# tohinz/multiple-objects-gan

Measured on AMD Instinct MI355X. Metric: images/sec per G+D train step, 256x256 coco-attngan, higher is better.
Workload: dtype f32

## Files before the change

include/mogan_hip.h:

```cpp
#ifndef MOGAN_HIP_H
#define MOGAN_HIP_H

#include <stddef.h>
#include <stdint.h>

#ifdef __cplusplus
extern "C" {
#endif

typedef struct ihipStream_t* hipStream_t;

#define MOGAN_ERR_SHAPE (-1)
#define MOGAN_ERR_LAUNCH (-2)
#define MOGAN_ERR_WS (-3)

#define MOGAN_ACT_NONE 0
#define MOGAN_ACT_RELU 1
#define MOGAN_ACT_LRELU 2
#define MOGAN_ACT_GLU 3
#define MOGAN_ACT_TANH 4
#define MOGAN_ACT_SIGMOID 5

int mogan_abi_version(void);
int mogan_gemm_set_split_target(int blocks);
// ... 82 lines not shown

size_t mogan_pk_panel_bytes(int B, int C, int HW);
int mogan_deep_block_eligible(int B, int Cin, int Hs, int Ws, int Cout, int KH, int KW, int stride, int ph, int pw, int act,
                              int groups);
int mogan_deep_conv_bn_act_fwd(const float* x, const void* xpanel, const void* wpk, const float* gamma, const float* beta,
                               float* rmean, float* rvar, float* y, float* stats, float* z, void* zpanel, int B, int Cin, int Hs,
                               int Ws, int Cout, int KH, int KW, int stride, int ph, int pw, float eps, float momentum, int act,
                               float slope, int groups, void* ws, size_t ws_bytes, hipStream_t stream);
int mogan_deep_conv_bn_act_bwd(const float* dz, const float* y, const float* stats, const float* gamma, const float* beta,
                               const void* wpk_dgrad, float* dy, float* dgamma, float* dbeta, int accumulate, float* dx, int B,
                               int Cin, int Hs, int Ws, int Cout, int KH, int KW, int stride, int ph, int pw, int act, float slope,
                               int groups, void* ws, size_t ws_bytes, hipStream_t stream);

typedef struct MoganPkArgs {
    const void* wpk; const void* panel; float* raw;
    int B, M;
    int Cp, CGp, cg0;
    int PH, PW, outH, outW;
    int KH, KW, stride, ph, pw, dgrad;
    int nsplit;
} MoganPkArgs;
#define MOGAN_TAIL_MAXSRC 3
typedef struct MoganTailArgs {
    const float* src[MOGAN_TAIL_MAXSRC]; long long src_bs[MOGAN_TAIL_MAXSRC]; long long src_slab[MOGAN_TAIL_MAXSRC];
    int src_nsplit[MOGAN_TAIL_MAXSRC]; int nsrc;
    const float* add; long long add_bs;
    const float* mask; long long mask_bs;
    const float* scale; const float* shift;
    int relu, box;
    float* dst; long long dst_bs;
    void* panel; int CGp, cg0;
    int B, n, H, W;
} MoganTailArgs;
int mogan_pk_group(int n, MoganPkArgs* args, hipStream_t stream);
int mogan_panel_tail_group(int n, const MoganTailArgs* args, hipStream_t stream);

size_t mogan_upconv3x3_ws_bytes(int Cout, int Cin);
int mogan_upconv3x3_k4(const float* w, float* k4, int Cout, int Cin, hipStream_t stream);
int mogan_upconv3x3_k4_group(int n, const float* const* w, float* const* k4, const int* Cout, const int* Cin, hipStream_t stream);
int mogan_upconv3x3_fwd(const float* x, const float* w, float* y, int B, int Cin, int Hs, int Ws, int Cout, void* ws,
                        size_t ws_bytes, hipStream_t stream);
int mogan_upconv3x3_dgrad(const float* dy, const float* w, float* dx, int B, int Cin, int Hs, int Ws, int Cout, void* ws,
                          size_t ws_bytes, hipStream_t stream);
int mogan_upconv3x3_wgrad(const float* dy, const float* x, float* dw, int B, int Cin, int Hs, int Ws, int Cout,
                          int accumulate, void* ws, size_t ws_bytes, hipStream_t stream);
int mogan_down2_sum(const float* du, float* dx, int planes, int H, int W, hipStream_t stream);

int mogan_bmm(const float* a, const float* b, float* c, int batch, int M, int N, int K, long long sAb, long long sAm,
              long long sAk, long long sBb, long long sBk, long long sBn, long long sCb, long long sCm, long long sCn,
              int accumulate, void* ws, size_t ws_bytes, hipStream_t stream);

size_t mogan_bn_ws_bytes(int B, int C, int HW);
int mogan_bn_stats(const float* x, int B, int C, int HW, float eps, float momentum, float* mean, float* invstd,
                   float* running_mean, float* running_var, void* ws, size_t ws_bytes, hipStream_t stream);
int mogan_bn_act_fwd(const float* x, const float* mean, const float* invstd, const float* gamma, const float* beta,
                     const float* residual, float* y, int B, int C, int HW, int act, float slope, hipStream_t stream);
int mogan_bn_running_update(const float* mean, const float* invstd, float* running_mean, float* running_var, int C, long long n,
                            float eps, float momentum, hipStream_t stream);

int mogan_bn_act_fwd_fused(const float* x, const float* gamma, const float* beta, const float* residual, float* running_mean,
                           float* running_var, float* mean, float* invstd, float* y, int B, int C, int HW, int act, float slope,
                           float eps, float momentum, void* ws, size_t ws_bytes, hipStream_t stream);
int mogan_bn_act_grouped_eligible(int G, int B, int C, int HW);
int mogan_bn_act_grouped_fwd(const float* x, const float* gamma, const float* beta, float* running_mean, float* running_var, float* mean,
                             float* invstd, float* y, int G, int B, int C, int HW, int act, float slope, float eps, float momentum,
                             hipStream_t stream);
int mogan_bn_act_grouped_bwd(const float* x, const float* dy, const float* mean, const float* invstd, const float* gamma, const float* beta,
// ... 131 lines not shown
```

multiple-objects-gan_amd/csrc/mogan_pgemm.hip:

```cpp
#include <hip/hip_runtime.h>
#include <stdint.h>
#include <stdlib.h>
#include <algorithm>
#include "../../include/mogan_hip.h"
#include "mogan_internal.h"
#include "mogan_mma.h"
#include <type_traits>
#ifndef PK_NSET
#define PK_NSET 3
#endif
#define PK_TRIP (PK_NSET == 2 ? 2 : 6)

namespace {

typedef float f32x16 __attribute__((ext_vector_type(16)));

struct PkP {
    const unsigned char* A;
    const unsigned char* P;
    float* C; float* ws;
    int M, N, K;
    int Mt, KS;
    unsigned long long a_cls_stride;
    unsigned a_bytes, p_bytes;
    int ntile, kt_per, nsplit;
    long long slab;
    int accumulate;
    int dgrad, ncls;
    int Cc, CG;
    int CGp, cg0;
    int PH, PW;
    int RH, RW;
    int s, ph, pw, nkw;
    int outH, outW;
    int gx, gy;
};

__device__ __forceinline__ unsigned xcd_order(unsigned L, unsigned total) {
    const unsigned k = L & 7u, j = L >> 3, q = total >> 3, r = total & 7u;
    return k * q + (k < r ? k : r) + j;
}

__device__ __forceinline__ uint4 ldg16(__amdgpu_buffer_rsrc_t r, unsigned off, bool ok) {
    return __builtin_bit_cast(uint4, __builtin_amdgcn_raw_buffer_load_b128(r, ok ? off : 0xFFFFFFF0u, 0, 0));
}

template <int TM, int TN, int WM = 4>
__device__ __forceinline__ void pgemm_body(const PkP& p, unsigned V, const unsigned nblk) {
    constexpr int WN = 4 / WM;
    constexpr int BM = WM * TM * 32, BN = WN * TN * 32, RS = 208;
    constexpr int NCH = BN * 12 / 256;
    __shared__ __attribute__((aligned(16))) unsigned char Bs[2][BN * RS];

    const int tid = threadIdx.x, lane = tid & 63, wave = tid >> 6;
    const int wm = wave % WM, wn = wave / WM;
    V = xcd_order(V, nblk);
    const unsigned bx = V % p.gx; V /= p.gx;
    const unsigned cls = V % p.ncls; V /= p.ncls;
    const unsigned by = V % p.gy;
    const int sp = V / p.gy;
    const int n0 = bx * BN, m0 = by * BM;
    const int t_beg = sp * p.kt_per, t_end = min(p.ntile, t_beg + p.kt_per);

    const __amdgpu_buffer_rsrc_t rA = __builtin_amdgcn_make_buffer_rsrc((void*)(p.A + cls * p.a_cls_stride), (short)0,
                                                                         (int)p.a_bytes, 0x00020000);
    const __amdgpu_buffer_rsrc_t rP = __builtin_amdgcn_make_buffer_rsrc((void*)p.P, (short)0, (int)p.p_bytes, 0x00020000);

    int py = 0, px = 0, kh0 = 0, kw0 = 0;
    if (p.dgrad) { py = cls / p.s; px = cls % p.s; kh0 = (py + p.ph) % p.s; kw0 = (px + p.pw) % p.s; }
    const int RHW = p.RH * p.RW;
    int ry[NCH], rx[NCH]; unsigned pb[NCH]; unsigned ldso[NCH], cho[NCH]; bool rok[NCH];
#pragma unroll
    for (int i = 0; i < NCH; ++i) {
        const int c = tid + 256 * i, row = c / 12, ch = c - row * 12;
        const int n = n0 + row;
        rok[i] = n < p.N;
        const int nn = rok[i] ? n : 0;
        const int img = nn / RHW, rem = nn - img * RHW;
        const int r = rem / p.RW, cc = rem - r * p.RW;
        if (p.dgrad) { ry[i] = (r * p.s + py + p.ph - kh0) / p.s; rx[i] = (cc * p.s + px + p.pw - kw0) / p.s; }
        else { ry[i] = r * p.s - p.ph; rx[i] = cc * p.s - p.pw; }
        pb[i] = (unsigned)img * (unsigned)(p.PH * p.PW);
        ldso[i] = row * RS + ch * 16;
        cho[i] = ch * 16;
    }
// ... 116 lines not shown
        }
    }

    const bool split = p.nsplit > 1;
    float* __restrict__ slab = p.ws + (size_t)sp * p.slab;
    const bool addc = !split && p.accumulate;
    const size_t cms = (size_t)p.outH * p.outW;
#pragma unroll
    for (int tb = 0; tb < TN; ++tb) {
        const int n = n0 + (wn * TN + tb) * 32 + (lane & 31);
        const bool nok = n < p.N;
        const int nn = nok ? n : 0;
        const int img = nn / RHW, rem = nn - img * RHW;
        const int r = rem / p.RW, cc = rem - r * p.RW;
        const size_t pos = p.dgrad ? (size_t)(r * p.s + py) * p.outW + (cc * p.s + px) : (size_t)rem;
        const size_t cbase = (size_t)img * p.M * cms + pos;
#pragma unroll
        for (int ta = 0; ta < TM; ++ta) {
#pragma unroll
            for (int r16 = 0; r16 < 16; ++r16) {
                const int m = m0 + (wm * TM + ta) * 32 + (r16 & 3) + 8 * (r16 >> 2) + 4 * (lane >> 5);
                if (nok && m < p.M) {
                    float v = acc[ta][tb][r16];
                    float* dst = (split ? slab : p.C) + cbase + (size_t)m * cms;
                    if (addc) v += *dst;
                    *dst = v;
                }
            }
        }
    }
}

template <int TM, int TN, int OCC>
__global__ __launch_bounds__(256, OCC) void pgemm_kernel(const PkP p) { pgemm_body<TM, TN>(p, blockIdx.x, gridDim.x); }

constexpr int PK_MAXG = 8;
struct PkGroup { PkP p[PK_MAXG]; unsigned end[PK_MAXG]; int n; };

template <int TM, int TN, int OCC, int WM>
__global__ __launch_bounds__(256, OCC) void pgemm_group_kernel(const PkGroup g) {
    int pi = 0;
#pragma unroll
    for (int i = 0; i < PK_MAXG - 1; ++i) if (i + 1 < g.n && blockIdx.x >= g.end[i]) pi = i + 1;
    const unsigned start = pi ? g.end[pi - 1] : 0u;
    pgemm_body<TM, TN, WM>(g.p[pi], blockIdx.x - start, g.end[pi] - start);
}

__global__ __launch_bounds__(256) void apack_kernel(const float* __restrict__ x, unsigned char* __restrict__ P, int Bn, int C,
                                                    int HW) {
    __shared__ float L[32][65];
    const int tid = threadIdx.x;
    const long long Q = (long long)Bn * HW;
    const long long q0 = (long long)blockIdx.x * 64;
    const int c0 = blockIdx.y * 32;
#pragma unroll
    for (int j = 0; j < 8; ++j) {
        const int e = tid + 256 * j, cl = e >> 6, ql = e & 63;
        const long long q = q0 + ql;
        float v = 0.f;
        if (q < Q) {
            const long long img = q / HW, pix = q - img * HW;
            v = x[(img * C + c0 + cl) * HW + pix];
        }
        L[cl][ql] = v;
    }
    __syncthreads();
    const int ql = tid >> 2, g8 = tid & 3;
    const long long q = q0 + ql;
    if (q >= Q) return;
    uint32_t w[3][4];
#pragma unroll
    for (int j = 0; j < 4; ++j) x6_split2(L[g8 * 8 + 2 * j][ql], L[g8 * 8 + 2 * j + 1][ql], w[0][j], w[1][j], w[2][j]);
    unsigned char* d = P + ((size_t)q * (C >> 5) + blockIdx.y) * 192 + g8 * 16;
#pragma unroll
    for (int pl = 0; pl < 3; ++pl) *(uint4*)(d + pl * 64) = make_uint4(w[pl][0], w[pl][1], w[pl][2], w[pl][3]);
}

struct WpackP { const float* w; unsigned char* A; int Cout, Cin, KH, KW, s, ph, pw, dgrad, M, Cc, Mt, KS; unsigned long long cls_stride; };
// ... 377 lines not shown
           (act == MOGAN_ACT_NONE || act == MOGAN_ACT_RELU || act == MOGAN_ACT_LRELU);
}

static inline long long cdiv(long long a, long long b) { return (a + b - 1) / b; }
static inline size_t up256(size_t v) { return (v + 255) & ~(size_t)255; }

static int g_pk_force = 0;

struct PkGeom { int ncls, nkh, nkw, M, Cc, K, Mt, KS; unsigned long long cls_bytes; };

static bool pk_geom(int Cout, int Cin, int KH, int KW, int s, int dgrad, PkGeom& g) {
    if (Cout <= 0 || Cin <= 0 || KH <= 0 || KW <= 0 || s <= 0) return false;
    if (!dgrad) {
        if (Cin % 32) return false;
        g.ncls = 1; g.nkh = KH; g.nkw = KW; g.M = Cout; g.Cc = Cin;
    } else {
        if (Cout % 32 || KH % s || KW % s) return false;
        g.ncls = s * s; g.nkh = KH / s; g.nkw = KW / s; g.M = Cin; g.Cc = Cout;
    }
    if (KH * KW > 25) return false;
    g.K = g.nkh * g.nkw * g.Cc;
    g.Mt = (int)cdiv(g.M, 32); g.KS = g.K / 16;
    g.cls_bytes = (unsigned long long)g.Mt * g.KS * 3072ull;
    return g.cls_bytes < (1ull << 32);
}

struct PkCfg { int tm, tn; };
static const PkCfg kPk[] = {{1, 2}, {1, 4}, {2, 2}};
enum { NPK = 3 };
static int g_pk_cfg = -1, g_pk_split = 0;
#ifndef PK_OCC12
#define PK_OCC12 3
#endif
#ifndef PK_G64_OCC
#define PK_G64_OCC 2
#endif
static int g_pk_group_tile = -1;
static inline int a_prof_mode(int dgrad) { return dgrad ? 11 : 10; }

template <int TM, int TN, int OCC>
static void launch_pk(unsigned blocks, hipStream_t st, const PkP& p) {
    hipLaunchKernelGGL((pgemm_kernel<TM, TN, OCC>), dim3(blocks), dim3(256), 0, st, p);
}

static int run_pk(PkP& p, void* ws, size_t ws_bytes, int prof_mode, hipStream_t st, bool keep_slabs = false) {
    int best = 0; double bestw = 1e300;
    for (int c = 0; c < NPK; ++c) {
        const int bm = 128 * kPk[c].tm, bn = 32 * kPk[c].tn;
        double w = (double)cdiv(p.M, bm) * bm * (double)cdiv(p.N, bn) * bn;
        w *= c == 0 ? 1.0 : 1.15;
        if (w < bestw * 0.999) { bestw = w; best = c; }
    }
    if (g_pk_cfg >= 0) best = g_pk_cfg;
    const int bm = 128 * kPk[best].tm, bn = 32 * kPk[best].tn;
    p.gx = (int)cdiv(p.N, bn); p.gy = (int)cdiv(p.M, bm);
    const long long tiles = (long long)p.gx * p.gy * p.ncls;
    const long long c_numel = (long long)p.slab;
    int nsplit = 1;
    const int target = mogan_split_target(st);
    if (tiles < target && p.ntile >= 8) {
        nsplit = (int)cdiv(target, tiles);
        nsplit = std::min(nsplit, p.ntile / 4);
        if (nsplit < 1) nsplit = 1;
    }
    if (g_pk_split > 0) nsplit = std::min(g_pk_split, p.ntile);
    if (nsplit > 1) {
        const long long fit = ws ? (long long)(ws_bytes / (sizeof(float) * (size_t)c_numel)) : 0;
        if (fit < 2) nsplit = 1; else nsplit = (int)std::min<long long>(nsplit, fit);
    }
    p.kt_per = (int)cdiv(cdiv(p.ntile, nsplit), PK_TRIP) * PK_TRIP;
    p.nsplit = (int)cdiv(p.ntile, p.kt_per);
    p.ws = (float*)ws;
    const long long blocks = tiles * p.nsplit;
    if (blocks <= 0 || blocks > 0x7fffffff) return MOGAN_ERR_SHAPE;
    const double flops = 2.0 * (double)p.M * (double)p.N * p.ncls * (double)p.K;
    mogan_prof_begin(prof_mode, best, flops, p.M, p.N * p.ncls, p.K, st);
    switch (best) {
        case 1: launch_pk<1, 4, 2>((unsigned)blocks, st, p); break;
        case 2: launch_pk<2, 2, 2>((unsigned)blocks, st, p); break;
        default: launch_pk<1, 2, PK_OCC12>((unsigned)blocks, st, p); break;
    }
    mogan_prof_end(1, st);
    if (p.nsplit > 1 && !keep_slabs) mogan_splitk_reduce_dense((const float*)ws, p.C, c_numel, p.nsplit, p.accumulate, st);
    return hipGetLastError() == hipSuccess ? 0 : MOGAN_ERR_LAUNCH;
}

static int apack(const float* x, unsigned char* P, int B, int C, int HW, hipStream_t st) {
    const long long Q = (long long)B * HW;
    hipLaunchKernelGGL(apack_kernel, dim3((unsigned)cdiv(Q, 64), (unsigned)(C / 32)), dim3(256), 0, st, x, P, B, C, HW);
    return 0;
}

}

extern "C" {

int mogan_pk_debug_force(int take_all, int cfg, int split) {
    g_pk_force = take_all; g_pk_cfg = (cfg >= 0 && cfg < NPK) ? cfg : -1; g_pk_split = split > 0 ? split : 0;
    return 0;
}

int mogan_pk_conv_eligible(int B, int Cin, int Hs, int Ws, int Cout, int KH, int KW, int stride, int ph, int pw, int dgrad) {
    PkGeom g;
    if (B <= 0 || Hs <= 0 || Ws <= 0 || !pk_geom(Cout, Cin, KH, KW, stride, dgrad, g)) return 0;
    const int OH = (Hs + 2 * ph - KH) / stride + 1, OW = (Ws + 2 * pw - KW) / stride + 1;
    if (OH <= 0 || OW <= 0) return 0;
    if (dgrad && (Hs % stride || Ws % stride)) return 0;
    const long long pix = dgrad ? (long long)B * OH * OW : (long long)B * Hs * Ws;
    if (pix * g.Cc * 6 >= (1ll << 32)) return 0;
    if (g_pk_force) return 1;
    const int rows_hw = dgrad ? (Hs / stride) * (Ws / stride) : OH * OW;
    return rows_hw <= 64 && g.K >= 1024 && g.M >= 128;
}

size_t mogan_pk_weight_bytes(int Cout, int Cin, int KH, int KW, int stride, int dgrad) {
    PkGeom g;
    if (!pk_geom(Cout, Cin, KH, KW, stride, dgrad, g)) return 0;
    return (size_t)g.cls_bytes * g.ncls;
}

int mogan_pk_weight_pack(const float* w, void* wpk, int Cout, int Cin, int KH, int KW, int stride, int ph, int pw, int dgrad,
                         hipStream_t stream) {
    PkGeom g;
    if (!w || !wpk || !pk_geom(Cout, Cin, KH, KW, stride, dgrad, g)) return MOGAN_ERR_SHAPE;
    WpackP p{};
    p.w = w; p.A = (unsigned char*)wpk; p.Cout = Cout; p.Cin = Cin; p.KH = KH; p.KW = KW; p.s = dgrad ? stride : 1;
    p.ph = ph; p.pw = pw; p.dgrad = dgrad; p.M = g.M; p.Cc = g.Cc; p.Mt = g.Mt; p.KS = g.KS; p.cls_stride = g.cls_bytes;
    if (g.Cc % 16) return MOGAN_ERR_SHAPE;
    const size_t lds = (size_t)KH * KW * 32 * 17 * sizeof(float);
    hipLaunchKernelGGL(wpack_kernel, dim3((unsigned)g.Mt, (unsigned)(g.Cc / 16)), dim3(256), lds, stream, p);
    return hipGetLastError() == hipSuccess ? 0 : MOGAN_ERR_LAUNCH;
// ... 95 lines not shown
    Kpad = (int)((npix + 31) / 32 * 32);
    R = (long long)Cin * KH * KW;
    abytes = up256((size_t)((Cout + 31) / 32) * 32 * Kpad * 6);
    pbytes = up256((size_t)R * Kpad * 6);
    return pbytes < (1ull << 32) && (long long)Cout * R < (1ll << 31);
}

int mogan_pk_wgrad_eligible(int B, int Cin, int Hs, int Ws, int Cout, int KH, int KW, int stride, int ph, int pw, size_t ws_bytes) {
    int OH, OW, Kpad; long long R; size_t ab, pb;
    if (!wgrad_pk_sizes(B, Cin, Hs, Ws, Cout, KH, KW, stride, ph, pw, OH, OW, Kpad, R, ab, pb)) return 0;
    if (ab + pb > ws_bytes) return 0;
    if (g_pk_force) return 1;
    return OH * OW <= 64 && Kpad >= 512 && (long long)Cout * R >= (16ll << 20);
}

int mogan_conv2d_wgrad_pk(const float* dy, const float* x, float* dw, int B, int Cin, int Hs, int Ws, int Cout, int KH, int KW,
                          int stride, int ph, int pw, int accumulate, void* ws, size_t ws_bytes, hipStream_t stream) {
    int OH, OW, Kpad; long long R; size_t ab, pb;
    if (!dy || !x || !dw || !wgrad_pk_sizes(B, Cin, Hs, Ws, Cout, KH, KW, stride, ph, pw, OH, OW, Kpad, R, ab, pb)) return MOGAN_ERR_SHAPE;
    if (!ws || ab + pb > ws_bytes) return MOGAN_ERR_WS;
    unsigned char* A = (unsigned char*)ws;
    unsigned char* P = A + ab;
    const int Mt = (Cout + 31) / 32, KS = Kpad / 16, npix = B * OH * OW;
    hipLaunchKernelGGL(dypack_kernel, dim3((unsigned)cdiv((long long)Mt * KS * 64, 256)), dim3(256), 0, stream, dy, A, Cout, OH * OW,
                       npix, KS);
    XtP q{};
    q.x = x; q.P = P; q.Cin = Cin; q.Hs = Hs; q.Ws = Ws; q.KH = KH; q.KW = KW; q.s = stride; q.ph = ph; q.pw = pw; q.OH = OH; q.OW = OW;
    q.Npix = npix; q.KG = Kpad / 32; q.total = R * (Kpad / 8);
    hipLaunchKernelGGL(xtpack_kernel, dim3((unsigned)cdiv(q.total, 256)), dim3(256), 0, stream, q);
    return pk_fwd_from_panel(P, A, dw, 1, Kpad, (int)R, 1, Cout, 1, 1, 1, 0, 0, (char*)ws + ab + pb, ws_bytes - ab - pb, stream, false,
                             nullptr, accumulate, 9);
}

int mogan_pk_group(int n, MoganPkArgs* args, hipStream_t stream) {
    constexpr int env_tile = -1;
    g_pk_group_tile = env_tile;
    if (n <= 0 || n > PK_MAXG || !args) return MOGAN_ERR_SHAPE;
    PkGroup g{};
    g.n = n;
    long long end = 0; double flops = 0;
    double w128 = 0, w64 = 0;
    for (int i = 0; i < n; ++i) {
        const double N = (double)args[i].B * args[i].outH * args[i].outW, K = (double)args[i].KH * args[i].KW * args[i].Cp;
        w128 += (double)cdiv(args[i].M, 128) * 128 * (double)cdiv((long long)N, 64) * 64 * K;
        w64 += (double)cdiv(args[i].M, 64) * 64 * (double)cdiv((long long)N, 128) * 128 * K;
    }
    (void)w64; (void)w128;
    const int tile64 = g_pk_group_tile > 0 ? 1 : 0;
    const int bm = tile64 ? 64 : 128, bn = tile64 ? 128 : 64;
    for (int i = 0; i < n; ++i) {
        const MoganPkArgs& a = args[i];
        if (!a.wpk || !a.panel || !a.raw || a.B <= 0 || a.M <= 0 || a.Cp <= 0 || a.Cp % 32 || a.cg0 < 0 || a.cg0 + a.Cp / 32 > a.CGp ||
            a.KH <= 0 || a.KW <= 0 || a.KH * a.KW > 25 || a.stride <= 0 || (a.dgrad && a.stride != 1) || a.PH <= 0 || a.PW <= 0 ||
            a.outH <= 0 || a.outW <= 0 || a.nsplit <= 0)
            return MOGAN_ERR_SHAPE;
        const size_t pbytes = (size_t)a.B * a.PH * a.PW * a.CGp * 192;
        const long long slab = (long long)a.B * a.M * a.outH * a.outW;
        PkP& p = g.p[i];
        p.A = (const unsigned char*)a.wpk; p.P = (const unsigned char*)a.panel; p.C = a.raw; p.ws = a.raw;
        p.M = a.M; p.N = a.B * a.outH * a.outW; p.K = a.KH * a.KW * a.Cp; p.Mt = (int)cdiv(p.M, 32); p.KS = p.K / 16;
        const unsigned long long abytes = (unsigned long long)p.Mt * p.KS * 3072ull;
        if (pbytes >= (1ull << 32) || abytes >= (1ull << 32) || slab >= (1ll << 31)) return MOGAN_ERR_SHAPE;
        p.a_cls_stride = abytes; p.a_bytes = (unsigned)abytes; p.p_bytes = (unsigned)pbytes; p.ntile = p.K / 32; p.slab = slab;
        p.accumulate = 0; p.dgrad = a.dgrad; p.ncls = 1; p.Cc = a.Cp; p.CG = a.Cp / 32; p.CGp = a.CGp; p.cg0 = a.cg0;
        p.PH = a.PH; p.PW = a.PW; p.RH = a.outH; p.RW = a.outW; p.s = a.stride; p.ph = a.ph; p.pw = a.pw; p.nkw = a.KW;
        p.outH = a.outH; p.outW = a.outW;
        p.gx = (int)cdiv(p.N, bn); p.gy = (int)cdiv(p.M, bm);
        p.kt_per = (int)cdiv(cdiv(p.ntile, std::min(a.nsplit, p.ntile)), PK_TRIP) * PK_TRIP;
        while (cdiv(p.ntile, p.kt_per) > a.nsplit) p.kt_per += PK_TRIP;
        p.nsplit = (int)cdiv(p.ntile, p.kt_per);
        args[i].nsplit = p.nsplit;
        end += (long long)p.gx * p.gy * p.nsplit;
        if (end > 0x7fffffff) return MOGAN_ERR_SHAPE;
        g.end[i] = (unsigned)end;
        flops += 2.0 * (double)p.M * (double)p.N * (double)p.K;
    }
    mogan_prof_begin(a_prof_mode(args[0].dgrad), tile64, flops, g.p[0].M, g.p[0].N, g.p[0].K, stream);
    if (tile64) hipLaunchKernelGGL((pgemm_group_kernel<1, 2, PK_G64_OCC, 2>), dim3((unsigned)end), dim3(256), 0, stream, g);
    else hipLaunchKernelGGL((pgemm_group_kernel<1, 2, 3, 4>), dim3((unsigned)end), dim3(256), 0, stream, g);
    mogan_prof_end(1, stream);
    return hipGetLastError() == hipSuccess ? 0 : MOGAN_ERR_LAUNCH;
}

size_t mogan_pk_panel_bytes(int B, int C, int HW) { return (B > 0 && C > 0 && HW > 0) ? (size_t)B * HW * C * 6 : 0; }

int mogan_deep_block_eligible(int B, int Cin, int Hs, int Ws, int Cout, int KH, int KW, int stride, int ph, int pw, int act,
                              int groups) {
    if (groups < 1 || B <= 0 || B % groups) return 0;
    if (!mogan_pk_conv_eligible(B, Cin, Hs, Ws, Cout, KH, KW, stride, ph, pw, 0)) return 0;
    if (!mogan_pk_conv_eligible(B, Cin, Hs, Ws, Cout, KH, KW, stride, ph, pw, 1)) return 0;
    const int OH = (Hs + 2 * ph - KH) / stride + 1, OW = (Ws + 2 * pw - KW) / stride + 1;
    return tail_ok(B / groups, Cout, OH * OW, act, groups) ? 1 : 0;
}

int mogan_deep_conv_bn_act_fwd(const float* x, const void* xpanel, const void* wpk, const float* gamma, const float* beta,
                               float* rmean, float* rvar, float* y, float* stats, float* z, void* zpanel, int B, int Cin, int Hs,
                               int Ws, int Cout, int KH, int KW, int stride, int ph, int pw, float eps, float momentum, int act,
                               float slope, int groups, void* ws, size_t ws_bytes, hipStream_t stream) {
    if (B <= 0 || groups < 1 || B % groups || Cin <= 0 || Cin % 32 || Hs <= 0 || Ws <= 0 || stride <= 0) return MOGAN_ERR_SHAPE;
    const int OH = (Hs + 2 * ph - KH) / stride + 1, OW = (Ws + 2 * pw - KW) / stride + 1;
    if (OH <= 0 || OW <= 0 || !tail_ok(B / groups, Cout, OH * OW, act, groups) || !gamma || !beta || !y || !stats || !z)
        return MOGAN_ERR_SHAPE;
    char* w0 = (char*)ws; size_t wn = ws_bytes;
    if (!xpanel) {
        const size_t pbytes = up256((size_t)B * Hs * Ws * Cin * 6);
        if (!ws || ws_bytes < pbytes) return MOGAN_ERR_WS;
        apack(x, (unsigned char*)ws, B, Cin, Hs * Ws, stream);
        xpanel = ws; w0 += pbytes; wn -= pbytes;
    }
    int nsplit = 1;
    int rc = pk_fwd_from_panel(xpanel, wpk, y, B, Cin, Hs, Ws, Cout, KH, KW, stride, ph, pw, w0, wn, stream, true, &nsplit);
    if (rc) return rc;
// ... 36 lines not shown
```

multiple-objects-gan_amd/hip/lib.py:

```python
import contextlib
import ctypes
import os

import torch

_HERE = os.path.dirname(os.path.dirname(os.path.abspath(__file__)))
LIB_PATH = os.environ.get("MOGAN_LIB") or os.path.join(_HERE, "libmogan_hip.so")

P, I, F, L, Z = ctypes.c_void_p, ctypes.c_int, ctypes.c_float, ctypes.c_longlong, ctypes.c_size_t

SIGNATURES = {
    "mogan_abi_version": [],
    "mogan_gemm_set_split_target": [I],
    "mogan_stream_set_split_target": [P, I],
    "mogan_gemm_debug_force": [I, I],
    "mogan_gemm_group_min_tiles": [I],
    "mogan_mfma_form": [],
    "mogan_gemm_tune_set": [I, I, I, I, I, I, I],
    "mogan_gemm_tune_clear": [],
    "mogan_reserve_streams": [ctypes.c_int],
    "mogan_prof_enable": [I],
    "mogan_prof_collect": [P, I],
    "mogan_prof_dump": [ctypes.c_char_p],
    "mogan_conv2d_out_dims": [I, I, I, I, I, I, I, I, P, P],
# ... 54 lines not shown
    "mogan_scale": [P, F, P, L, P],
    "mogan_softmax_fwd": [P, P, P, L, I, L, F, P],
    "mogan_softmax_bwd": [P, P, P, P, L, I, L, F, P],
    "mogan_stn_fwd": [P, P, P, I, I, I, I, I, I, I, P],
    "mogan_stn_bwd": [P, P, P, I, I, I, I, I, I, I, P],
    "mogan_stn_fwd_ex": [P, P, P, I, I, I, I, I, I, I, I, I, I, P],
    "mogan_stn_bwd_ex": [P, P, P, I, I, I, I, I, I, I, I, I, I, P],
    "mogan_concat_fwd": [P, P, P, P, P, P, I, P, I, I, P],
    "mogan_concat_bwd": [P, P, P, P, P, P, P, I, I, I, P],
    "mogan_bbox_to_theta": [P, P, P, I, P],
    "mogan_attn_fwd": [P, P, P, P, P, I, I, I, I, I, P],
    "mogan_attn_bwd": [P, P, P, P, P, P, I, I, I, I, P],
    "mogan_bce_fwd": [P, F, F, P, I, I, P],
    "mogan_bce_bwd": [P, F, F, P, P, I, P],
    "mogan_bce_logits_fwd": [P, F, F, P, I, I, P],
    "mogan_bce_logits_bwd": [P, F, F, P, P, I, P],
    "mogan_kl_fwd": [P, P, P, I, P],
    "mogan_kl_bwd": [P, P, P, P, P, I, P],
    "mogan_reparam_fwd": [P, P, P, P, I, P],
    "mogan_reparam_bwd": [P, P, P, P, P, I, P],
    "mogan_maxpool_fwd": [P, P, P, I, I, I, I, I, P],
    "mogan_maxpool_bwd": [P, P, P, I, I, I, I, I, P],
    "mogan_avgpool_fwd": [P, P, I, I, I, I, I, I, P],
    "mogan_avgpool_bwd": [P, P, I, I, I, I, I, I, P],
    "mogan_bilinear_fwd": [P, P, I, I, I, I, I, P],
    "mogan_bilinear_bwd": [P, P, I, I, I, I, I, P],
    "mogan_adam_step": [P, P, P, P, P, L, F, F, F, F, I, P, I, F, F, P],
    "mogan_conv2d_affine_fwd_ex": [P, L, P, P, P, P, L, P, L, I] + [I] * 11 + [P, Z, P],
    "mogan_conv2d_fwd_ex": [P, L, P, P, L, P, L, I] + [I] * 10 + [P, Z, P],
    "mogan_conv2d_dgrad_ex": [P, L, P, P, L, P, L, I] + [I] * 10 + [P, Z, P],
    "mogan_conv2d_affine_fwd_group": [I, P, P, Z, P],
    "mogan_conv2d_dgrad_group": [I, P, P, Z, P],
    "mogan_pk_group": [I, P, P],
    "mogan_panel_tail_group": [I, P, P],
    "mogan_maxpool_fwd_ex": [P, P, L, P, I, I, I, I, I, I, P],
    "mogan_maxpool_bwd_ex": [P, P, L, P, P, I, I, I, I, I, I, I, P],
    "mogan_avgpool_bwd_ex": [P, P, P, I, I, I, I, I, I, I, P],
    "mogan_copy_strided": [P, L, P, L, I, L, P],
    "mogan_relu_bwd": [P, P, P, L, I, P],
    "mogan_feed_crop_flip": [P, P, P, P, I, I, I, P],
    "mogan_feed_resample": [P, P, P, P, P, I, I, I, I, P],
    "mogan_damsm_words_fwd": [P, P, P, I, I, I, I, I, F, F, F, P, P, P, P, P, P],
    "mogan_damsm_words_bwd": [P, P, P, P, P, P, P, I, I, I, I, I, F, F, F, P, P, P],
    "mogan_damsm_ce_fwd": [P, P, P, I, I, P, P, P, P, P],
    "mogan_damsm_ce_bwd": [P, P, P, P, P, I, I, P, P],
    "mogan_damsm_sent_fwd": [P, P, I, I, I, F, F, P, P],
    "mogan_damsm_sent_bwd": [P, P, P, I, I, I, F, F, P, P],
    "mogan_damsm_words_bwd_text": [P, P, P, P, I, I, I, I, F, F, P, P],
    "mogan_damsm_sent_bwd_text": [P, P, P, I, I, I, F, F, P, P],
    "mogan_lstm_encoder_train_fwd": [P] * 10 + [F] + [P] * 6 + [I] * 6 + [P],
    "mogan_lstm_encoder_bwd": [P] * 10 + [I] * 3 + [P],
    "mogan_embedding_bwd": [P, P, P, P, F, P, I, I, I, I, I, P],
    "mogan_scalar_sum": [P, P, I, P, P],
    "mogan_scalar_scale": [P, P, I, P, P],
}


class ConvFwdArgs(ctypes.Structure):
    _fields_ = [("x", P), ("x_bstride", L), ("w", P), ("scale", P), ("shift", P), ("y", P), ("y_bstride", L), ("y2", P),
                ("y2_bstride", L), ("msplit", I)] + [(k, I) for k in ("B", "Cin", "Hs", "Ws", "Cout", "KH", "KW", "stride",
                                                                      "ph", "pw", "relu")]


class ConvDgradArgs(ctypes.Structure):
    _fields_ = [("dy", P), ("dy_bstride", L), ("w", P), ("dx", P), ("dx_bstride", L), ("relu_of", P), ("relu_bstride", L),
                ("accumulate", I)] + [(k, I) for k in ("B", "Cin", "Hs", "Ws", "Cout", "KH", "KW", "stride", "ph", "pw")]


class PkArgs(ctypes.Structure):
    _fields_ = [("wpk", P), ("panel", P), ("raw", P)] + [(k, I) for k in ("B", "M", "Cp", "CGp", "cg0", "PH", "PW", "outH", "outW",
                                                                       "KH", "KW", "stride", "ph", "pw", "dgrad", "nsplit")]


class TailArgs(ctypes.Structure):
    _fields_ = [("src", P * 3), ("src_bs", L * 3), ("src_slab", L * 3), ("src_nsplit", I * 3), ("nsrc", I), ("add", P), ("add_bs", L),
                ("mask", P), ("mask_bs", L), ("scale", P), ("shift", P), ("relu", I), ("box", I), ("dst", P), ("dst_bs", L),
                ("panel", P), ("CGp", I), ("cg0", I), ("B", I), ("n", I), ("H", I), ("W", I)]


_RESTYPE = {"mogan_bn_ws_bytes": Z, "mogan_upconv3x3_ws_bytes": Z, "mogan_pk_weight_bytes": Z, "mogan_pk_panel_bytes": Z,
            "mogan_wino_prep_bytes": Z, "mogan_conv_prep_bytes": Z}
_ERRORS = {-1: "MOGAN_ERR_SHAPE", -2: "MOGAN_ERR_LAUNCH", -3: "MOGAN_ERR_WS"}

_lib = None
_ws = {}
WORKSPACE_BYTES = int(os.environ.get("MOGAN_WS_MB", "256")) << 20


class MoganHipError(RuntimeError):
    pass


def load():
    global _lib
    if _lib is None:
        if not os.path.isfile(LIB_PATH):
            raise MoganHipError(
                "libmogan_hip.so is not built (%s). Run `python __graft_entry__.py` / "
                "`python multiple-objects-gan_amd/build.py`; there is no CPU fallback." % LIB_PATH)
        lib = ctypes.CDLL(LIB_PATH)
        for name, args in SIGNATURES.items():
            fn = getattr(lib, name)
            fn.argtypes = args
            fn.restype = _RESTYPE.get(name, I)
        _lib = lib
        _register_tuned(lib)
# ... 107 lines not shown
```

Measured before the change: 457.5.

## Add halo-staged implicit-GEMM body reusing LDS input tile across conv taps

Result: no change. 459.9, median of 6 (+0.5%).

```diff
diff --git a/include/mogan_hip.h b/include/mogan_hip.h
--- a/include/mogan_hip.h
+++ b/include/mogan_hip.h
@@ -138,7 +138,12 @@
     void* panel; int CGp, cg0;
     int B, n, H, W;
 } MoganTailArgs;
+typedef struct MoganPkPlan {
+    int body, tile_rows, gx, gy, blocks, slabs, lds_bytes;
+    int units, per, taps;
+} MoganPkPlan;
 int mogan_pk_group(int n, MoganPkArgs* args, hipStream_t stream);
+int mogan_pk_group_plan(int n, const MoganPkArgs* args, MoganPkPlan* plan);
 int mogan_panel_tail_group(int n, const MoganTailArgs* args, hipStream_t stream);
 
 size_t mogan_upconv3x3_ws_bytes(int Cout, int Cin);
diff --git a/multiple-objects-gan_amd/csrc/mogan_pgemm.hip b/multiple-objects-gan_amd/csrc/mogan_pgemm.hip
--- a/multiple-objects-gan_amd/csrc/mogan_pgemm.hip
+++ b/multiple-objects-gan_amd/csrc/mogan_pgemm.hip
@@ -46,11 +46,11 @@
 }
 
 template <int TM, int TN, int WM = 4>
-__device__ __forceinline__ void pgemm_body(const PkP& p, unsigned V, const unsigned nblk) {
+__device__ __forceinline__ void pgemm_body(const PkP& p, unsigned V, const unsigned nblk,
+                                           unsigned char (*__restrict__ Bs)[(4 / WM) * TN * 32 * 208]) {
     constexpr int WN = 4 / WM;
     constexpr int BM = WM * TM * 32, BN = WN * TN * 32, RS = 208;
     constexpr int NCH = BN * 12 / 256;
-    __shared__ __attribute__((aligned(16))) unsigned char Bs[2][BN * RS];
 
     const int tid = threadIdx.x, lane = tid & 63, wave = tid >> 6;
     const int wm = wave % WM, wn = wave / WM;
@@ -233,18 +233,191 @@
 }
 
 template <int TM, int TN, int OCC>
-__global__ __launch_bounds__(256, OCC) void pgemm_kernel(const PkP p) { pgemm_body<TM, TN>(p, blockIdx.x, gridDim.x); }
+__global__ __launch_bounds__(256, OCC) void pgemm_kernel(const PkP p) {
+    __shared__ __attribute__((aligned(16))) unsigned char Bs[2][TN * 32 * 208];
+    pgemm_body<TM, TN>(p, blockIdx.x, gridDim.x, Bs);
+}
+
+struct PkH {
+    int body;
+    int RWs, RHs, Zr, Zc;
+    int oy, ox, sgn;
+    int nkh, cg_per, B;
+};
+
+template <int WM>
+__device__ __forceinline__ void pgemm_halo_body(const PkP& p, const PkH& h, unsigned V, const unsigned nblk,
+                                                unsigned char* __restrict__ lds) {
+    constexpr int WN = 4 / WM, TN = 2 / WN, BM = WM * 32, BN = 64, RS = 208, MAXI = 5;
+    const int tid = threadIdx.x, lane = tid & 63;
+    const int wave = __builtin_amdgcn_readfirstlane(tid >> 6);
+    const int wm = wave % WM, wn = wave / WM;
+    V = xcd_order(V, nblk);
+    const unsigned bx = V % p.gx; V /= p.gx;
+    const unsigned by = V % p.gy;
+    const int sp = V / p.gy;
+    const int n0 = bx * BN, m0 = by * BM;
+    const int cg_beg = sp * h.cg_per, cg_end = min(p.CG, cg_beg + h.cg_per);
+    const int T = h.nkh * p.nkw;
+
+    const int RHW = p.RH * p.RW;
+    auto rbase = [&](int n) {
+        const int img = n / RHW, rem = n - img * RHW;
+        const int r = rem / p.RW, c = rem - r * p.RW;
+        return (img * h.RHs + r + h.oy + h.Zr) * h.RWs + c + h.ox + h.Zc;
+    };
+    const int span = (h.nkh - 1) * h.RWs + (p.nkw - 1);
+    const int b0 = rbase(n0);
+    const int lo = b0 - (h.sgn < 0 ? span : 0);
+    const int S = rbase(min(n0 + BN, p.N) - 1) - b0 + span + 1;
+
+    const __amdgpu_buffer_rsrc_t rA = __builtin_amdgcn_make_buffer_rsrc((void*)p.A, (short)0, (int)p.a_bytes, 0x00020000);
+    const __amdgpu_buffer_rsrc_t rP = __builtin_amdgcn_make_buffer_rsrc((void*)p.P, (short)0, (int)p.p_bytes, 0x00020000);
+
+    const int sq = tid >> 2, qd = tid & 3;
+    const unsigned pixb = (unsigned)p.CGp * 192u;
+    unsigned soff[MAXI];
+#pragma unroll
+    for (int i = 0; i < MAXI; ++i) {
+        const int s = sq + 64 * i, pos = lo + s;
+        const int row = pos / h.RWs, col = pos - row * h.RWs;
+        const int img = row / h.RHs, rr = row - img * h.RHs;
+        const bool ok = (int)(s < S) & (int)(col >= h.Zc) & (int)(rr >= h.Zr) & (int)(img < h.B);
+        const unsigned off = ((unsigned)((img * p.PH + rr - h.Zr) * p.PW + col - h.Zc)) * pixb + (unsigned)p.cg0 * 192u + (unsigned)qd * 16u;
+        soff[i] = ok ? off : 0xFFFF0000u;
+    }
+    auto stage_halo = [&](int cg) {
+        const unsigned goff = (unsigned)cg * 192u;
+        uint4 v[MAXI][3];
+#pragma unroll
+        for (int i = 0; i < MAXI; ++i)
+            if (i * 64 < S) {
+#pragma unroll
+                for (int q = 0; q < 3; ++q) v[i][q] = ldg16(rP, soff[i] + goff + (unsigned)q * 64u, true);
+            }
+#pragma unroll
+        for (int i = 0; i < MAXI; ++i)
+            if (sq + 64 * i < S) {
+#pragma unroll
+                for (int q = 0; q < 3; ++q) *(uint4*)(lds + (sq + 64 * i) * RS + qd * 16 + q * 64) = v[i][q];
+            }
+    };
+
+    if (m0 + wm * 32 >= p.M) {
+        for (int cg = cg_beg; cg < cg_end; ++cg) {
+            __syncthreads();
+            stage_halo(cg);
+            __syncthreads();
+        }
+        return;
+    }
+
+    int pixo[TN];
+#pragma unroll
+    for (int tb = 0; tb < TN; ++tb) {
+        const int n = min(n0 + (wn * TN + tb) * 32 + (lane & 31), p.N - 1);
+        pixo[tb] = (rbase(n) - lo) * RS + (lane >> 5) * 16;
+    }
+    const unsigned abase = (unsigned)((m0 >> 5) + wm) * (unsigned)p.KS * 3072u + (unsigned)lane * 16u;
+    const int dxB = h.sgn * RS, dyB = h.sgn * h.RWs * RS;
+
+    f32x16 acc[TN];
+#pragma unroll
+    for (int b = 0; b < TN; ++b)
+#pragma unroll
+        for (int r = 0; r < 16; ++r) acc[b][r] = 0.f;
+
+    uint4 ra[3][2][3];
+    int tapA = 0, cgA = cg_beg;
+    auto load_a = [&](uint4 (&r)[2][3]) {
+        const bool live = cgA < cg_end;
+        const unsigned ks = (unsigned)(tapA * p.CG + cgA) * 2u;
+#pragma unroll
+        for (int s2 = 0; s2 < 2; ++s2)
+#pragma unroll
+            for (int pl = 0; pl < 3; ++pl) r[s2][pl] = ldg16(rA, abase + ((ks + s2) * 3u + pl) * 1024u, live);
+        if (++tapA == T) { tapA = 0; ++cgA; }
+    };
+    auto read_b = [&](int toff, int s2, int tb) {
+        X6Frag f;
+#pragma unroll
+        for (int pl = 0; pl < 3; ++pl)
+            f.p[pl] = __builtin_bit_cast(mma_bf16x8, *(const uint4*)(lds + pixo[tb] + toff + pl * 64 + s2 * 32));
+        return f;
+    };
+    auto compute = [&](const uint4 (&r)[2][3], int toff) {
+        X6Frag fb = read_b(toff, 0, 0);
+#pragma unroll
+        for (int s2 = 0; s2 < 2; ++s2) {
+            X6Frag fa;
+#pragma unroll
+            for (int pl = 0; pl < 3; ++pl) fa.p[pl] = __builtin_bit_cast(mma_bf16x8, r[s2][pl]);
+#pragma unroll
+            for (int tb = 0; tb < TN; ++tb) {
+                const X6Frag cur = fb;
+                if (tb + 1 < TN) fb = read_b(toff, s2, tb + 1);
+                else if (s2 == 0) fb = read_b(toff, 1, 0);
+#pragma unroll
+                for (int term = 0; term < 6; ++term) acc[tb] = x6_mfma(fa, cur, term, acc[tb]);
+            }
+        }
+    };
+    int tapC = 0, tbC = 0, cgC = cg_beg, toffC = 0;
+    auto item = [&](auto SET) {
+        constexpr int St = decltype(SET)::value;
+        const bool live = cgC < cg_end;
+        if (tapC == 0 && live) {
+            __syncthreads();
+            stage_halo(cgC);
+            __syncthreads();
+        }
+        load_a(ra[(St + 2) % 3]);
+        compute(ra[St], live ? toffC : 0);
+        toffC += dxB;
+        if (++tbC == p.nkw) { tbC = 0; toffC += dyB - p.nkw * dxB; }
+        if (++tapC == T) { tapC = 0; tbC = 0; toffC = 0; ++cgC; }
+    };
+    load_a(ra[0]);
+    load_a(ra[1]);
+    using I0 = std::integral_constant<int, 0>; using I1 = std::integral_constant<int, 1>; using I2 = std::integral_constant<int, 2>;
+    const int nitem = (cg_end - cg_beg) * T;
+    for (int j = 0; j < nitem; j += 3) {
+        item(I0{});
+        item(I1{});
+        item(I2{});
+    }
+
+    const bool split = p.nsplit > 1;
+    float* __restrict__ out = split ? p.ws + (size_t)sp * p.slab : p.C;
+    const size_t cms = (size_t)p.outH * p.outW;
+#pragma unroll
+    for (int tb = 0; tb < TN; ++tb) {
+        const int n = n0 + (wn * TN + tb) * 32 + (lane & 31);
+        const bool nok = n < p.N;
+        const int nn = nok ? n : 0;
+        const int img = nn / RHW, rem = nn - img * RHW;
+        const size_t cbase = (size_t)img * p.M * cms + (size_t)rem;
+#pragma unroll
+        for (int r16 = 0; r16 < 16; ++r16) {
+            const int m = m0 + wm * 32 + (r16 & 3) + 8 * (r16 >> 2) + 4 * (lane >> 5);
+            if (nok && m < p.M) out[cbase + (size_t)m * cms] = acc[tb][r16];
+        }
+    }
+}
 
 constexpr int PK_MAXG = 8;
-struct PkGroup { PkP p[PK_MAXG]; unsigned end[PK_MAXG]; int n; };
-
-template <int TM, int TN, int OCC, int WM>
+struct PkGroup { PkP p[PK_MAXG]; PkH h[PK_MAXG]; unsigned end[PK_MAXG]; int n; };
+
+template <int OCC>
 __global__ __launch_bounds__(256, OCC) void pgemm_group_kernel(const PkGroup g) {
+    extern __shared__ __attribute__((aligned(16))) unsigned char pk_lds[];
     int pi = 0;
 #pragma unroll
     for (int i = 0; i < PK_MAXG - 1; ++i) if (i + 1 < g.n && blockIdx.x >= g.end[i]) pi = i + 1;
     const unsigned start = pi ? g.end[pi - 1] : 0u;
-    pgemm_body<TM, TN, WM>(g.p[pi], blockIdx.x - start, g.end[pi] - start);
+    const int body = g.h[pi].body;
+    if (body == 1) pgemm_halo_body<2>(g.p[pi], g.h[pi], blockIdx.x - start, g.end[pi] - start, pk_lds);
+    else pgemm_body<1, 2, 4>(g.p[pi], blockIdx.x - start, g.end[pi] - start, (unsigned char (*)[64 * 208])pk_lds);
 }
 
 __global__ __launch_bounds__(256) void apack_kernel(const float* __restrict__ x, unsigned char* __restrict__ P, int Bn, int C,
@@ -688,10 +861,7 @@
 #ifndef PK_OCC12
 #define PK_OCC12 3
 #endif
-#ifndef PK_G64_OCC
-#define PK_G64_OCC 2
-#endif
-static int g_pk_group_tile = -1;
+static int g_pk_group_old = 0;
 static inline int a_prof_mode(int dgrad) { return dgrad ? 11 : 10; }
 
 template <int TM, int TN, int OCC>
@@ -752,7 +922,8 @@
 extern "C" {
 
 int mogan_pk_debug_force(int take_all, int cfg, int split) {
-    g_pk_force = take_all; g_pk_cfg = (cfg >= 0 && cfg < NPK) ? cfg : -1; g_pk_split = split > 0 ? split : 0;
+    g_pk_force = take_all & 1; g_pk_group_old = (take_all >> 1) & 1;
+    g_pk_cfg = (cfg >= 0 && cfg < NPK) ? cfg : -1; g_pk_split = split > 0 ? split : 0;
     return 0;
 }
 
@@ -914,52 +1085,104 @@
                              nullptr, accumulate, 9);
 }
 
+}
+
+namespace {
+constexpr int PK_HALO_MAXPOS = 315;
+constexpr int PK_TAPMAJOR_LDS = 2 * 64 * 208;
+
+static int pk_plan_member(const MoganPkArgs& a, PkP& p, PkH& h, MoganPkPlan& o) {
+    if (a.B <= 0 || a.M <= 0 || a.Cp <= 0 || a.Cp % 32 || a.cg0 < 0 || a.CGp <= 0 || a.cg0 + a.Cp / 32 > a.CGp || a.KH <= 0 ||
+        a.KW <= 0 || a.KH * a.KW > 25 || a.stride <= 0 || (a.dgrad && a.stride != 1) || a.PH <= 0 || a.PW <= 0 || a.outH <= 0 ||
+        a.outW <= 0 || a.nsplit <= 0)
+        return MOGAN_ERR_SHAPE;
+    const unsigned long long pbytes = (unsigned long long)a.B * a.PH * a.PW * a.CGp * 192ull;
+    const long long slab = (long long)a.B * a.M * a.outH * a.outW;
+    p = PkP{}; h = PkH{};
+    p.M = a.M; p.N = a.B * a.outH * a.outW; p.K = a.KH * a.KW * a.Cp; p.Mt = (int)cdiv(p.M, 32); p.KS = p.K / 16;
+    const unsigned long long abytes = (unsigned long long)p.Mt * p.KS * 3072ull;
+    if (pbytes >= (1ull << 32) || abytes >= (1ull << 32) || slab >= (1ll << 31)) return MOGAN_ERR_SHAPE;
+    p.a_cls_stride = abytes; p.a_bytes = (unsigned)abytes; p.p_bytes = (unsigned)pbytes; p.ntile = p.K / 32; p.slab = slab;
+    p.accumulate = 0; p.dgrad = a.dgrad; p.ncls = 1; p.Cc = a.Cp; p.CG = a.Cp / 32; p.CGp = a.CGp; p.cg0 = a.cg0;
+    p.PH = a.PH; p.PW = a.PW; p.RH = a.outH; p.RW = a.outW; p.s = a.stride; p.ph = a.ph; p.pw = a.pw; p.nkw = a.KW;
+    p.outH = a.outH; p.outW = a.outW;
+    p.gx = (int)cdiv(p.N, 64);
+
+    h.sgn = a.dgrad ? -1 : 1; h.oy = a.dgrad ? a.ph : -a.ph; h.ox = a.dgrad ? a.pw : -a.pw; h.nkh = a.KH; h.B = a.B;
+    const int ylo = h.oy + std::min(0, h.sgn * (a.KH - 1)), yhi = a.outH - 1 + h.oy + std::max(0, h.sgn * (a.KH - 1));
+    const int xlo = h.ox + std::min(0, h.sgn * (a.KW - 1)), xhi = a.outW - 1 + h.ox + std::max(0, h.sgn * (a.KW - 1));
+    h.Zr = std::max(0, std::max(-ylo, yhi - (a.PH - 1))); h.Zc = std::max(0, std::max(-xlo, xhi - (a.PW - 1)));
+    h.RHs = a.PH + h.Zr; h.RWs = a.PW + h.Zc;
+    bool halo = !g_pk_group_old && a.stride == 1 && a.KH * a.KW > 1 && a.outH <= h.RHs && a.outW <= h.RWs &&
+                pbytes <= 0xFFFF0000ull && a.CGp * 192 < 0xF000;
+    int smax = 0;
+    if (halo) {
+        const int RHW = a.outH * a.outW, span = (a.KH - 1) * h.RWs + (a.KW - 1);
+        auto rbase = [&](int n) {
+            const int img = n / RHW, rem = n - img * RHW, r = rem / a.outW, c = rem - r * a.outW;
+            return (img * h.RHs + r) * h.RWs + c;
+        };
+        for (int n0 = 0; n0 < p.N; n0 += 64) smax = std::max(smax, rbase(std::min(n0 + 64, p.N) - 1) - rbase(n0) + span + 1);
+        halo = smax <= PK_HALO_MAXPOS;
+    }
+    const int rows = halo ? 64 : 128;
+    h.body = halo ? 1 : 0;
+    p.gy = (int)cdiv(p.M, rows);
+    int units, per;
+    if (halo) {
+        units = p.CG;
+        per = (int)cdiv(units, std::min(a.nsplit, units));
+        h.cg_per = per; p.kt_per = per * a.KH * a.KW;
+    } else {
+        units = p.ntile;
+        per = (int)cdiv(cdiv(units, std::min(a.nsplit, units)), PK_TRIP) * PK_TRIP;
+        while (cdiv(units, per) > a.nsplit) per += PK_TRIP;
+        p.kt_per = per;
+    }
+    p.nsplit = (int)cdiv(units, per);
+    const long long blocks = (long long)p.gx * p.gy * p.nsplit;
+    if (blocks > 0x7fffffff) return MOGAN_ERR_SHAPE;
+    o.body = halo ? 1 : 0; o.tile_rows = rows; o.gx = p.gx; o.gy = p.gy; o.slabs = p.nsplit; o.blocks = (int)blocks;
+    o.lds_bytes = halo ? smax * 208 : PK_TAPMAJOR_LDS; o.units = units; o.per = per; o.taps = a.KH * a.KW;
+    return 0;
+}
+}
+
+extern "C" {
+
+int mogan_pk_group_plan(int n, const MoganPkArgs* args, MoganPkPlan* plan) {
+    if (n <= 0 || n > PK_MAXG || !args || !plan) return MOGAN_ERR_SHAPE;
+    for (int i = 0; i < n; ++i) {
+        PkP p; PkH h;
+        const int rc = pk_plan_member(args[i], p, h, plan[i]);
+        if (rc) return rc;
+    }
+    return 0;
+}
+
 int mogan_pk_group(int n, MoganPkArgs* args, hipStream_t stream) {
-    constexpr int env_tile = -1;
-    g_pk_group_tile = env_tile;
     if (n <= 0 || n > PK_MAXG || !args) return MOGAN_ERR_SHAPE;
     PkGroup g{};
     g.n = n;
     long long end = 0; double flops = 0;
-    double w128 = 0, w64 = 0;
-    for (int i = 0; i < n; ++i) {
-        const double N = (double)args[i].B * args[i].outH * args[i].outW, K = (double)args[i].KH * args[i].KW * args[i].Cp;
-        w128 += (double)cdiv(args[i].M, 128) * 128 * (double)cdiv((long long)N, 64) * 64 * K;
-        w64 += (double)cdiv(args[i].M, 64) * 64 * (double)cdiv((long long)N, 128) * 128 * K;
-    }
-    (void)w64; (void)w128;
-    const int tile64 = g_pk_group_tile > 0 ? 1 : 0;
-    const int bm = tile64 ? 64 : 128, bn = tile64 ? 128 : 64;
+    int lds = 0;
     for (int i = 0; i < n; ++i) {
         const MoganPkArgs& a = args[i];
-        if (!a.wpk || !a.panel || !a.raw || a.B <= 0 || a.M <= 0 || a.Cp <= 0 || a.Cp % 32 || a.cg0 < 0 || a.cg0 + a.Cp / 32 > a.CGp ||
-            a.KH <= 0 || a.KW <= 0 || a.KH * a.KW > 25 || a.stride <= 0 || (a.dgrad && a.stride != 1) || a.PH <= 0 || a.PW <= 0 ||
-            a.outH <= 0 || a.outW <= 0 || a.nsplit <= 0)
-            return MOGAN_ERR_SHAPE;
-        const size_t pbytes = (size_t)a.B * a.PH * a.PW * a.CGp * 192;
-        const long long slab = (long long)a.B * a.M * a.outH * a.outW;
+        if (!a.wpk || !a.panel || !a.raw) return MOGAN_ERR_SHAPE;
+        MoganPkPlan pl;
+        const int rc = pk_plan_member(a, g.p[i], g.h[i], pl);
+        if (rc) return rc;
         PkP& p = g.p[i];
         p.A = (const unsigned char*)a.wpk; p.P = (const unsigned char*)a.panel; p.C = a.raw; p.ws = a.raw;
-        p.M = a.M; p.N = a.B * a.outH * a.outW; p.K = a.KH * a.KW * a.Cp; p.Mt = (int)cdiv(p.M, 32); p.KS = p.K / 16;
-        const unsigned long long abytes = (unsigned long long)p.Mt * p.KS * 3072ull;
-        if (pbytes >= (1ull << 32) || abytes >= (1ull << 32) || slab >= (1ll << 31)) return MOGAN_ERR_SHAPE;
-        p.a_cls_stride = abytes; p.a_bytes = (unsigned)abytes; p.p_bytes = (unsigned)pbytes; p.ntile = p.K / 32; p.slab = slab;
-        p.accumulate = 0; p.dgrad = a.dgrad; p.ncls = 1; p.Cc = a.Cp; p.CG = a.Cp / 32; p.CGp = a.CGp; p.cg0 = a.cg0;
-        p.PH = a.PH; p.PW = a.PW; p.RH = a.outH; p.RW = a.outW; p.s = a.stride; p.ph = a.ph; p.pw = a.pw; p.nkw = a.KW;
-        p.outH = a.outH; p.outW = a.outW;
-        p.gx = (int)cdiv(p.N, bn); p.gy = (int)cdiv(p.M, bm);
-        p.kt_per = (int)cdiv(cdiv(p.ntile, std::min(a.nsplit, p.ntile)), PK_TRIP) * PK_TRIP;
-        while (cdiv(p.ntile, p.kt_per) > a.nsplit) p.kt_per += PK_TRIP;
-        p.nsplit = (int)cdiv(p.ntile, p.kt_per);
         args[i].nsplit = p.nsplit;
-        end += (long long)p.gx * p.gy * p.nsplit;
+        end += pl.blocks;
         if (end > 0x7fffffff) return MOGAN_ERR_SHAPE;
         g.end[i] = (unsigned)end;
+        lds = std::max(lds, pl.lds_bytes);
         flops += 2.0 * (double)p.M * (double)p.N * (double)p.K;
     }
-    mogan_prof_begin(a_prof_mode(args[0].dgrad), tile64, flops, g.p[0].M, g.p[0].N, g.p[0].K, stream);
-    if (tile64) hipLaunchKernelGGL((pgemm_group_kernel<1, 2, PK_G64_OCC, 2>), dim3((unsigned)end), dim3(256), 0, stream, g);
-    else hipLaunchKernelGGL((pgemm_group_kernel<1, 2, 3, 4>), dim3((unsigned)end), dim3(256), 0, stream, g);
+    mogan_prof_begin(a_prof_mode(args[0].dgrad), 0, flops, g.p[0].M, g.p[0].N, g.p[0].K, stream);
+    hipLaunchKernelGGL((pgemm_group_kernel<3>), dim3((unsigned)end), dim3(256), (size_t)lds, stream, g);
     mogan_prof_end(1, stream);
     return hipGetLastError() == hipSuccess ? 0 : MOGAN_ERR_LAUNCH;
 }
diff --git a/multiple-objects-gan_amd/hip/lib.py b/multiple-objects-gan_amd/hip/lib.py
--- a/multiple-objects-gan_amd/hip/lib.py
+++ b/multiple-objects-gan_amd/hip/lib.py
@@ -110,6 +110,7 @@
     "mogan_conv2d_affine_fwd_group": [I, P, P, Z, P],
     "mogan_conv2d_dgrad_group": [I, P, P, Z, P],
     "mogan_pk_group": [I, P, P],
+    "mogan_pk_group_plan": [I, P, P],
     "mogan_panel_tail_group": [I, P, P],
     "mogan_maxpool_fwd_ex": [P, P, L, P, I, I, I, I, I, I, P],
     "mogan_maxpool_bwd_ex": [P, P, L, P, P, I, I, I, I, I, I, I, P],
@@ -150,6 +151,10 @@
                                                                        "KH", "KW", "stride", "ph", "pw", "dgrad", "nsplit")]
 
 
+class PkPlan(ctypes.Structure):
+    _fields_ = [(k, I) for k in ("body", "tile_rows", "gx", "gy", "blocks", "slabs", "lds_bytes", "units", "per", "taps")]
+
+
 class TailArgs(ctypes.Structure):
     _fields_ = [("src", P * 3), ("src_bs", L * 3), ("src_slab", L * 3), ("src_nsplit", I * 3), ("nsrc", I), ("add", P), ("add_bs", L),
                 ("mask", P), ("mask_bs", L), ("scale", P), ("shift", P), ("relu", I), ("box", I), ("dst", P), ("dst_bs", L),
```
